# lab-oak/oak

Measured on AMD Instinct MI355X. Metric: turn-steps/s (batched playouts), higher is better.
Workload: dtype u16

## Files before the change

### include/oakgpu.h

```cpp
#ifndef OAKGPU_H
#define OAKGPU_H
#include <stddef.h>
#include <stdint.h>

#ifdef __cplusplus
extern "C" {
#endif

#define OAKGPU_BATTLE_SIZE 384
#define OAKGPU_DURATIONS_SIZE 8
#define OAKGPU_ACTIONS_SIZE 16
#define OAKGPU_MAX_CHOICES 9
#define OAKGPU_TEAMS_SIZE 60

typedef struct oakgpu_ctx oakgpu_ctx;
typedef struct oakgpu_net oakgpu_net;

int oakgpu_create(oakgpu_ctx **out, int device);
void oakgpu_destroy(oakgpu_ctx *ctx);
const char *oakgpu_last_error(void);
int oakgpu_set_stream(oakgpu_ctx *ctx, void *hip_stream);
void *oakgpu_get_stream(oakgpu_ctx *ctx);
int oakgpu_synchronize(oakgpu_ctx *ctx);
int oakgpu_set_kernel_timing(oakgpu_ctx *ctx, int on);
int oakgpu_get_leaf_kernel_ms(oakgpu_ctx *ctx, float ms[3]);
int oakgpu_set_playouts_per_lane(oakgpu_ctx *ctx, int k);
int oakgpu_set_regroup(oakgpu_ctx *ctx, int rounds, int suspend_below, int shrink);
int oakgpu_set_tail_pack(oakgpu_ctx *ctx, int below, int waves, int lanes);
int oakgpu_set_queue_order(oakgpu_ctx *ctx, int on);
int oakgpu_set_spread(oakgpu_ctx *ctx, int lanes);
int oakgpu_set_migration(oakgpu_ctx *ctx, int mode, int long_steps, int adopters);
int oakgpu_set_migration_window(oakgpu_ctx *ctx, int window);
int oakgpu_set_standstill_skip(oakgpu_ctx *ctx, int on);
#define OAKGPU_MOVE_CARRY_DEFAULT 32
int oakgpu_set_move_carry(oakgpu_ctx *ctx, int below);
#define OAKGPU_CTL_FAST_FORWARDED 44
#define OAKGPU_CTL_SKIPPED_STEPS 45
int oakgpu_get_queue_counters(oakgpu_ctx *ctx, uint32_t *out64);
int oakgpu_device_count(void);

int oakgpu_rollout_dev(oakgpu_ctx *ctx, const uint8_t *battles, const uint8_t *durations,
                       const uint8_t *results_in, uint8_t *prng_state, uint32_t n, uint32_t max_steps,
                       int prep, uint8_t *results_out, uint32_t *steps_out, float *values_out,
                       uint8_t *battles_out, uint8_t *durations_out);
int oakgpu_rollout(oakgpu_ctx *ctx, const uint8_t *battles, const uint8_t *durations,
                   const uint8_t *results_in, uint8_t *prng_state, uint32_t n, uint32_t max_steps, int prep,
                   uint8_t *results_out, uint32_t *steps_out, float *values_out, uint8_t *battles_out,
                   uint8_t *durations_out);

typedef struct {
  const uint8_t *battles, *durations, *results_in;
  uint8_t *prng_state;
  uint32_t n;
  uint8_t *results_out;
  uint32_t *steps_out;
  float *values_out;
  uint8_t *battles_out, *durations_out;
} oakgpu_rollout_batch;
// ... 434 lines not shown
```

### oak_amd/_lib.py

```python
import ctypes as C
import os

_HERE = os.path.dirname(os.path.abspath(__file__))
LIB_PATH = os.environ.get("OAKGPU_LIB") or os.path.join(_HERE, "liboakgpu.so")

SYMBOLS = [
    "oakgpu_create", "oakgpu_destroy", "oakgpu_last_error", "oakgpu_set_stream", "oakgpu_get_stream", "oakgpu_synchronize", "oakgpu_set_kernel_timing", "oakgpu_get_leaf_kernel_ms", "oakgpu_set_playouts_per_lane", "oakgpu_set_regroup", "oakgpu_set_tail_pack", "oakgpu_set_queue_order", "oakgpu_queue_order", "oakgpu_set_spread", "oakgpu_set_migration", "oakgpu_set_migration_window", "oakgpu_set_standstill_skip", "oakgpu_set_move_carry", "oakgpu_get_queue_counters",
    "oakgpu_device_count", "oakgpu_rollout_dev", "oakgpu_rollout", "oakgpu_rollout_group_dev", "oakgpu_rollout_group",
    "oakgpu_mt19937_fill", "oakgpu_rollout_draws_dev", "oakgpu_rollout_shared_device", "oakgpu_update_dev", "oakgpu_update",
    "oakgpu_choices_dev", "oakgpu_choices", "oakgpu_init_battles_dev", "oakgpu_init_battles",
    "oakgpu_set_ou_pools", "oakgpu_random_ou_battles_dev",
    "oakgpu_net_load", "oakgpu_net_load_memory", "oakgpu_net_free", "oakgpu_net_shape", "oakgpu_net_set_main_precision", "oakgpu_net_main_precision", "oakgpu_net_policy_form",
    "oakgpu_net_load_discrete", "oakgpu_net_load_discrete_memory", "oakgpu_net_is_discrete", "oakgpu_leaf_eval_discrete_raw_dev",
    "oakgpu_leaf_eval_dev", "oakgpu_leaf_eval", "oakgpu_leaf_eval_cached_dev", "oakgpu_leaf_cache_last_count", "oakgpu_leaf_embed_forms", "oakgpu_leaf_eval_policy_dev", "oakgpu_leaf_eval_policy",
    "oakgpu_heap_create", "oakgpu_heap_destroy", "oakgpu_heap_empty", "oakgpu_heap_clear", "oakgpu_heap_kind", "oakgpu_heap_nodes", "oakgpu_heap_update",
    "oakgpu_heap_root_stats", "oakgpu_heap_child_stats", "oakgpu_search_heap", "oakgpu_search_agent_heap", "oakgpu_heap_check_shards", "oakgpu_heap_selftest",
    "oakgpu_tree_step_dev", "oakgpu_search", "oakgpu_search_many", "oakgpu_search_agent", "oakgpu_agent_networks_clear", "oakgpu_bandit_replay", "oakgpu_bandit_select_run", "oakgpu_solve_matrix",
    "oakgpu_segment_mean_dev", "oakgpu_comm_unique_id", "oakgpu_comm_create", "oakgpu_comm_destroy", "oakgpu_all_gather_dev",
    "oakgpu_root_steps_create", "oakgpu_root_steps_destroy", "oakgpu_root_steps_launch_dev", "oakgpu_root_steps_capacity", "oakgpu_root_steps_reserve",
    "oakgpu_endless_battle_check", "oakgpu_frames_size", "oakgpu_frames_write", "oakgpu_frames_read", "oakgpu_selfplay_game", "oakgpu_selfplay_games", "oakgpu_poke_engine_eval_dev", "oakgpu_poke_engine_eval",
    "oakgpu_replay_index", "oakgpu_replay_records_dev", "oakgpu_replay_records", "oakgpu_engine_switches",
    "oakgpu_corpus_create", "oakgpu_corpus_destroy", "oakgpu_corpus_info", "oakgpu_frames_encode_dev", "oakgpu_frames_sample_dev", "oakgpu_encode_battles_dev",
    "oakgpu_frames_encode", "oakgpu_frames_sample",
    "oakgpu_corpus_frame_bases", "oakgpu_corpus_chunks", "oakgpu_corpus_states_dev", "oakgpu_corpus_states", "oakgpu_corpus_inference_dev", "oakgpu_corpus_loss_dev",
    "oakgpu_corpus_inference", "oakgpu_corpus_evaluate",
    "oakgpu_party_table_create", "oakgpu_party_table_destroy", "oakgpu_party_table_fill_dev", "oakgpu_party_table_fill", "oakgpu_leaf_eval_table_dev",
    "oakgpu_leaf_eval_policy_table_dev", "oakgpu_party_table_last_misses", "oakgpu_party_table_rows", "oakgpu_party_table_width", "oakgpu_party_key", "oakgpu_party_variant",
    "oakgpu_set_search_party_table", "oakgpu_search_party_table_stats", "oakgpu_leaf_eval_table", "oakgpu_leaf_eval_policy_table",
    "oakgpu_policy_games_dev", "oakgpu_policy_games", "oakgpu_policy_games_last_stats",
    "oakgpu_forest_create", "oakgpu_forest_destroy", "oakgpu_forest_check", "oakgpu_forest_search_dev", "oakgpu_forest_search", "oakgpu_forest_nodes",
# ... 137 lines not shown
                          "(hipcc --offload-arch=gfx950); there is no CPU fallback")
    lib = C.CDLL(LIB_PATH)
    vp, u32, u64, i32 = C.c_void_p, C.c_uint32, C.c_uint64, C.c_int
    lib.oakgpu_create.argtypes = [C.POINTER(vp), i32]
    lib.oakgpu_destroy.argtypes = [vp]
    lib.oakgpu_destroy.restype = None
    lib.oakgpu_last_error.restype = C.c_char_p
    lib.oakgpu_set_stream.argtypes = [vp, vp]
    lib.oakgpu_get_stream.argtypes = [vp]
    lib.oakgpu_get_stream.restype = vp
    lib.oakgpu_synchronize.argtypes = [vp]
    lib.oakgpu_set_kernel_timing.argtypes = [vp, i32]
    lib.oakgpu_get_leaf_kernel_ms.argtypes = [vp, C.POINTER(C.c_float)]
    lib.oakgpu_set_playouts_per_lane.argtypes = [vp, i32]
    lib.oakgpu_set_regroup.argtypes = [vp, i32, i32, i32]
    lib.oakgpu_set_tail_pack.argtypes = [vp, i32, i32, i32]
    lib.oakgpu_set_queue_order.argtypes = [vp, i32]
    lib.oakgpu_queue_order.argtypes = [vp, C.POINTER(RolloutBatch), u32, vp, C.POINTER(u32)]
    lib.oakgpu_set_spread.argtypes = [vp, i32]
    lib.oakgpu_set_migration.argtypes = [vp, i32, i32, i32]
    lib.oakgpu_set_migration_window.argtypes = [vp, i32]
    lib.oakgpu_set_standstill_skip.argtypes = [vp, i32]
    lib.oakgpu_set_move_carry.argtypes = [vp, i32]
    lib.oakgpu_get_queue_counters.argtypes = [vp, vp]
    lib.oakgpu_rollout_dev.argtypes = [vp, vp, vp, vp, vp, u32, u32, i32, vp, vp, vp, vp, vp]
    lib.oakgpu_rollout.argtypes = [vp, vp, vp, vp, vp, u32, u32, i32, vp, vp, vp, vp, vp]
    lib.oakgpu_rollout_group_dev.argtypes = [vp, C.POINTER(RolloutBatch), u32, u32, i32]
    lib.oakgpu_rollout_group.argtypes = [vp, C.POINTER(RolloutBatch), u32, u32, i32]
    lib.oakgpu_mt19937_fill.argtypes = [u32, u64, vp, C.c_size_t]
    lib.oakgpu_rollout_draws_dev.argtypes = [vp, vp, u32, vp, u32, vp, u32, vp, u32, vp, u32, u32, i32, vp, vp, vp, vp, vp, vp]
    lib.oakgpu_rollout_shared_device.argtypes = [vp, vp, vp, C.c_uint8, vp, u32, u32, u32, i32, vp, vp, vp, vp, vp, vp, vp]
    lib.oakgpu_poke_engine_eval_dev.argtypes = [vp, vp, u32, C.c_float, vp, vp]
    lib.oakgpu_poke_engine_eval.argtypes = [vp, vp, u32, C.c_float, vp, vp]
    lib.oakgpu_tree_step_dev.argtypes = [vp, vp, vp, vp, vp, vp, u32, u32, vp, vp, vp, vp, vp]
    lib.oakgpu_search.argtypes = [vp, vp, vp, vp, C.c_uint8, C.POINTER(SearchParams), C.POINTER(SearchOutput)]
    lib.oakgpu_heap_create.argtypes = [C.POINTER(vp)]
    lib.oakgpu_heap_destroy.argtypes = [vp]
    lib.oakgpu_heap_destroy.restype = None
    lib.oakgpu_heap_empty.argtypes = [vp]
    lib.oakgpu_heap_clear.argtypes = [vp]
    lib.oakgpu_heap_clear.restype = None
    lib.oakgpu_heap_kind.argtypes = [vp]
    lib.oakgpu_heap_nodes.argtypes = [vp]
    lib.oakgpu_heap_nodes.restype = u64
    lib.oakgpu_heap_update.argtypes = [vp, C.c_uint8, C.c_uint8, vp]
    lib.oakgpu_heap_root_stats.argtypes = [vp, i32, vp, vp, vp, vp]
# ... 146 lines not shown
```

### oak_amd/csrc/gen1_regs.hpp

```cpp
#pragma once
#include "gen1_device.hpp"

namespace oak {

#ifdef OAKGPU_SITE_PROFILE
static __device__ unsigned long long g_site_prof[32 * 4];
__device__ __forceinline__ unsigned long long *site_lds() {
  __shared__ unsigned long long s_prof[32 * 4];
  return s_prof;
}
__device__ __forceinline__ void site_zero() {
  unsigned long long *p = site_lds();
  for (int i = threadIdx.x; i < 32 * 4; i += blockDim.x) p[i] = 0;
  __syncthreads();
}
__device__ __forceinline__ void site_flush() {
  __syncthreads();
  unsigned long long *p = site_lds();
  for (int i = threadIdx.x; i < 32 * 4; i += blockDim.x) if (p[i]) atomicAdd(&g_site_prof[i], p[i]);
}
__device__ __forceinline__ void site_add(int id, long long dt) {
  const uint64_t ex = __ballot(1);
  const uint32_t lane = __lane_id();
  if ((ex & ((1ull << lane) - 1)) == 0) {
// ... 33 lines not shown
struct SideR {
  uint32_t a0, a1, a2;
  uint32_t bo;
  uint32_t vlo, vhi;
  uint32_t m01, m23;
  uint32_t p0, p1, p2, p3, p4, p5;
  uint32_t o0, o1;
  uint32_t dur;
  uint32_t misc;
};

#define OAK_FOR_SIDE_FIELDS(X) X(a0) X(a1) X(a2) X(bo) X(vlo) X(vhi) X(m01) X(m23) X(p0) X(p1) X(p2) X(p3) X(p4) X(p5) X(o0) X(o1) X(dur) X(misc)

__device__ __forceinline__ void swap_sides(SideR &a, SideR &b) {
#define X(f) asm("v_swap_b32 %0, %1" : "+v"(a.f), "+v"(b.f));
  OAK_FOR_SIDE_FIELDS(X)
#undef X
}
__device__ __forceinline__ void cswap_sides(bool c, SideR &a, SideR &b) {
#define X(f) { uint32_t t = c ? b.f : a.f; b.f = c ? a.f : b.f; a.f = t; }
  OAK_FOR_SIDE_FIELDS(X)
#undef X
}

template <int STRIDE, bool TRACK_ACTIONS, bool GIN_LDS = false>
struct EngineR {
  lds_u32 *m;
  Tables T;
  SideR S, F;
  uint64_t actS, actF;
#ifdef OAKGPU_SITE_PROFILE
  int prof_k = 0;
#endif
  uint64_t rng;
  uint32_t turn, last_damage;
  uint32_t lm;

  static constexpr int PARTY_WORDS = 24;
  template <bool L, class Dummy = void> struct GinPtr { typedef const uint32_t *type; };
  template <class Dummy> struct GinPtr<true, Dummy> { typedef const lds_u32 *type; };
  typedef typename GinPtr<GIN_LDS>::type gin_t;
  gin_t gin;
  __device__ __forceinline__ uint4 gin4(int off) const {
    typedef uint32_t v4 __attribute__((ext_vector_type(4)));
    if constexpr (GIN_LDS) { const v4 t = *(const OAK_LDS v4 *)(gin + off); return make_uint4(t.x, t.y, t.z, t.w); }
    else return *(const uint4 *)(gin + off);
// ... 155 lines not shown
#pragma unroll
    for (uint32_t sd = 0; sd < 2; ++sd)
#pragma unroll
      for (uint32_t i = 0; i < 6; ++i) {
        const uint32_t d2 = gdw(sd, i, 2), d3 = gdw(sd, i, 3), d4 = gdw(sd, i, 4), d5 = gdw(sd, i, 5);
        set_pw(sd, i, 0, pack_pp(d2, d3, d4));
        set_pw(sd, i, 1, (d4 >> 16) | ((d5 & 0xFF) << 16));
      }
    { const uint4 v = gin4(36); S.a0 = v.x; S.a1 = v.y; S.a2 = v.z; S.bo = v.w; }
    { const uint4 v = gin4(40); S.vlo = v.x; S.vhi = v.y; S.m01 = v.z; S.m23 = v.w; }
    S.o0 = gin[44]; S.o1 = gin[45];
    F.a0 = gin[82]; F.a1 = gin[83];
    { const uint4 v = gin4(84); F.a2 = v.x; F.bo = v.y; F.vlo = v.z; F.vhi = v.w; }
    { const uint4 v = gin4(88); F.m01 = v.x; F.m23 = v.y; F.o0 = v.z; F.o1 = v.w; }
    { const uint4 v = gin4(92); turn = v.x & 0xFFFF; last_damage = v.x >> 16; lm = v.y; rng = (uint64_t)v.z | ((uint64_t)v.w << 32); }
    S.dur = dur0; F.dur = dur1;
    S.misc = 0; F.misc = 1u << 8;
    actS = actF = 0;
    alive_from_lds(S);
    alive_from_lds(F);
    load_stored(S);
    load_stored(F);
  }
  __device__ __forceinline__ void store_battle_global(uint8_t *battle384) {
    if (order0(S) != 0) writeback_stored(S);
    if (order0(F) != 0) writeback_stored(F);
    uint32_t *g = (uint32_t *)battle384;
#pragma unroll
    for (uint32_t sd = 0; sd < 2; ++sd)
#pragma unroll
      for (uint32_t i = 0; i < 6; ++i) {
        const uint32_t pp = pw(sd, i, 0), hs = pw(sd, i, 1);
        uint32_t *d = g + sd * 46 + i * 6;
        d[0] = gdw(sd, i, 0);
        d[1] = gdw(sd, i, 1);
        d[2] = (gdw(sd, i, 2) & 0x00FFFFFFu) | ((pp & 0xFF) << 24);
        d[3] = (gdw(sd, i, 3) & 0x00FF00FFu) | (((pp >> 8) & 0xFF) << 8) | (((pp >> 16) & 0xFF) << 24);
        d[4] = (gdw(sd, i, 4) & 0x000000FFu) | ((pp >> 24) << 8) | ((hs & 0xFFFF) << 16);
        d[5] = (gdw(sd, i, 5) & 0xFFFFFF00u) | ((hs >> 16) & 0xFF);
      }
    *(uint4 *)(g + 36) = make_uint4(S.a0, S.a1, S.a2, S.bo);
    *(uint4 *)(g + 40) = make_uint4(S.vlo, S.vhi, S.m01, S.m23);
    g[44] = S.o0; g[45] = S.o1;
    g[82] = F.a0; g[83] = F.a1;
    *(uint4 *)(g + 84) = make_uint4(F.a2, F.bo, F.vlo, F.vhi);
    *(uint4 *)(g + 88) = make_uint4(F.m01, F.m23, F.o0, F.o1);
    *(uint4 *)(g + 92) = make_uint4(turn | (last_damage << 16), lm, (uint32_t)rng, (uint32_t)(rng >> 32));
// ... 774 lines not shown
  __device__ __forceinline__ uint32_t end_turn() {
    turn += 1;
    if (turn >= 1000) return mk_result(R_TIE, 0, 0);
    return mk_result(0, C_MOVE, C_MOVE);
  }

  __device__ __forceinline__ void normalize() {
    const bool flipped = absp(S) != 0;
    cswap_sides(flipped, S, F);
    if constexpr (TRACK_ACTIONS) { uint64_t t = flipped ? actF : actS; actF = flipped ? actS : actF; actS = t; }
  }

  __device__ __forceinline__ uint32_t post_action(uint32_t choice, bool replace, bool residual) {
    OAK_SCOPE(PS_FAINT_RESIDUAL);
    if (replace) return 0;
    uint32_t r = 0;
    if ((choice & 3) != C_SWITCH) r = check_faint(F, S);
    if (r == 0) {
      if (residual) handle_residual();
      r = check_faint(S, F);
    }
    return r;
  }
  __device__ __forceinline__ uint32_t act_cheap(uint32_t choice) {
    const bool replace = hp(S) == 0;
    if ((choice & 3) == C_SWITCH) { OAK_SCOPE(PS_SWITCH_IN); switch_in(S, F, choice >> 2); }
    return post_action(choice, replace, false);
  }
  __device__ __forceinline__ uint32_t act_move(uint32_t choice) {
    OAK_T0(t_em);
    const bool replace = hp(S) == 0;
    uint32_t mslot = choice >> 2;
    if (last_sel(S) == M_Struggle) mslot = 0;
    else if (mslot == 0) mslot = lm_index(absp(S));
    OAK_T0(t_bm);
    const int r = before_move();
    OAK_T1(PS_BEFORE_MOVE, t_bm);
    if (r == BM_ERR) return mk_result(R_ERROR, 0, 0);
    if (r != BM_DONE) execute_selected(mslot, r == BM_SKIP_CAN, r == BM_SKIP_PP);
    OAK_T1(PS_EXEC_MOVE, t_em);
    OAK_T1K(PS_EXEC_MOVE_K0, t_em);
    return post_action(choice, replace, true);
  }

  __device__ __forceinline__ uint32_t turn_prologue(uint32_t cS, uint32_t cF, uint32_t &pc, uint32_t &qc) {
    if constexpr (TRACK_ACTIONS) { actS = 0; actF = 0; }
    if (turn == 0) {
      const bool aS = (S.misc & 63) != 0, aF = (F.misc & 63) != 0;
      const bool s_p1 = absp(S) == 0;
      if (!aS) return mk_result(aF ? (s_p1 ? R_LOSE : R_WIN) : R_TIE, 0, 0);
      if (!aF) return mk_result(s_p1 ? R_WIN : R_LOSE, 0, 0);
#pragma unroll 1
      for (int k = 0; k < 2; ++k) { switch_in(S, F, 1); swap_sides(S, F); }
      return end_turn();
    }
    OAK_T0(t_ord);
    select_move(S, cS);
    select_move(F, cF);
    bool f_first;
    {
      const uint32_t tS = cS & 3, tF = cF & 3;
      if (tS == C_PASS) f_first = true;
      else if (tF == C_PASS) f_first = false;
      else if ((tS == C_SWITCH) != (tF == C_SWITCH)) f_first = tS != C_SWITCH;
      else {
        const uint32_t mS = last_sel(S), mF = last_sel(F);
        bool decided = false;
        f_first = false;
        if (tS == C_MOVE) {
          if ((mS == M_QuickAttack) != (mF == M_QuickAttack)) { f_first = mS != M_QuickAttack; decided = true; }
          else if ((mS == M_Counter) != (mF == M_Counter)) { f_first = mS == M_Counter; decided = true; }
        }
        if (!decided) {
          const uint32_t sS = spe(S), sF = spe(F);
          if (sS == sF) {
            const bool p1 = rng_range(0, 2) == 0;
            act_set(true, AC_SPEEDTIE, 2, p1 ? 1 : 2);
            act_set(false, AC_SPEEDTIE, 2, p1 ? 1 : 2);
            f_first = p1 != (absp(S) == 0);
          } else f_first = sS < sF;
        }
      }
    }
    pc = f_first ? cF : cS;
    qc = f_first ? cS : cF;
    cswap_sides(f_first, S, F);
    if constexpr (TRACK_ACTIONS) { uint64_t t = f_first ? actF : actS; actF = f_first ? actS : actF; actS = t; }
    OAK_T1(PS_ORDER, t_ord);
    return 0;
  }
  __device__ __forceinline__ uint32_t turn_epilogue() {
    if ((S.vlo & V_BINDING) && attacks(S) == 0) clear_binding(S);
    if ((F.vlo & V_BINDING) && attacks(F) == 0) clear_binding(F);
    return end_turn();
  }
  __device__ __forceinline__ void next_actor() {
    swap_sides(S, F);
    if constexpr (TRACK_ACTIONS) { uint64_t t = actS; actS = actF; actF = t; }
  }

  __device__ __forceinline__ uint32_t act(uint32_t choice) { return (choice & 3) == C_MOVE ? act_move(choice) : act_cheap(choice); }
  __device__ __forceinline__ void hand_over(uint32_t &pc, uint32_t &qc) {
    next_actor();
    const uint32_t t = pc; pc = qc; qc = t;
  }
  __device__ __forceinline__ uint32_t turn_finish(uint32_t r) { return r ? r : turn_epilogue(); }

  __device__ uint32_t update_frame(uint32_t cS, uint32_t cF) {
    uint32_t pc = 0, qc = 0;
    uint32_t r = turn_prologue(cS, cF, pc, qc);
    if (r) return r;
#pragma unroll 1
    for (int k = 0; k < 2; ++k) {
      OAK_SET_K(*this, k);
      r = act(pc);
      const bool last = r != 0 || (qc & 3) == C_PASS;
      hand_over(pc, qc);
      if (last) break;
    }
    return turn_finish(r);
  }
  __device__ __forceinline__ uint32_t update(uint32_t c1, uint32_t c2) {
    const uint32_t r = update_frame(c1, c2);
    normalize();
// ... 171 lines not shown
```

### oak_amd/csrc/oakgpu.hip

```cpp
#include <hip/hip_runtime.h>
#include <stdint.h>
#include <stdio.h>
#include <stdlib.h>
#include <string.h>
#include <algorithm>
#include <random>
#include <mutex>
#include <string>
#include <type_traits>
#include <vector>

#include "../../include/oakgpu.h"
#include "gen1_device.hpp"
#include "gen1_regs.hpp"
#include "record_walk.hpp"
#include "oakgpu_internal.h"
#include "fast_prng.hpp"

namespace oak {
using namespace walk;

constexpr int STATE_WORDS = 96;
constexpr int TABLE_LDS_PAD = TABLE_PAD;

// ... 251 lines not shown
  if (a.battles_out) e.store_battle_global(a.battles_out + (size_t)lane * 384);
}

struct RoundArgs {
  const uint32_t *list_in;
  const uint32_t *n_in;
  uint32_t *list_out;
  uint32_t *count_out;
  uint8_t *sb;
  uint8_t *sd;
  uint8_t *sres;
  uint32_t suspend_below;
  uint32_t *queue;
  uint32_t lanes;
  const uint32_t *order;
  uint32_t *adopt_ctl;
  uint64_t *adopt_list;
  uint32_t epoch;
  uint32_t n_adopters;
  uint32_t long_steps;
  uint32_t no_skip;
  uint32_t *stats;
  uint32_t move_carry;
};

struct BatchDesc {
  const uint8_t *battles, *durations, *results_in;
  uint8_t *prng;
  uint8_t *results_out;
  uint32_t *steps_out;
  float *values_out;
  uint8_t *battles_out, *durations_out;
  uint32_t start, n;
};
constexpr int MAX_GROUP = 64;
struct GroupArgs {
  const BatchDesc *table;
  uint32_t count, total, max_steps;
  int prep;
};

struct ColdArgs {
  GroupArgs g;
  RoundArgs q;
  uint32_t starts[MAX_GROUP];
};
// ... 86 lines not shown
#define OAK_PRIO_STILL 24
#endif
constexpr uint32_t PRIO_STILL = OAK_PRIO_STILL;
template <int BLK, int WPS>
__global__ __launch_bounds__(BLK, WPS) void k_rollout_queue(GroupArgs g_in, RoundArgs q_in) {
  extern __shared__ __align__(16) uint8_t smem[];
  lds_u32 *party = (lds_u32 *)smem;
  using ER = EngineR<BLK, false>;
  Tables T = stage_default_tables((lds_u8 *)smem + ER::PARTY_WORDS * BLK * 4);
  lds_u32 *cold = (lds_u32 *)((lds_u8 *)smem + ER::PARTY_WORDS * BLK * 4 + TABLE_LDS_PAD);
  if (threadIdx.x == 0) {
    struct { GroupArgs g; RoundArgs q; } c{g_in, q_in};
    const uint32_t *src = (const uint32_t *)&c;
#pragma unroll
    for (uint32_t i = 0; i < offsetof(ColdArgs, starts) / 4; ++i) cold[i] = src[i];
  }
  for (uint32_t i = threadIdx.x; i < g_in.count; i += BLK) cold[offsetof(ColdArgs, starts) / 4 + i] = g_in.table[i].start;
  __syncthreads();
  const uint32_t tid = threadIdx.x, wl = tid & 63;
  constexpr uint32_t NONE = 0xFFFFFFFFu, DONE = 0xFFFFFFFEu;
#define COLD_U32(off) ((uint32_t)__builtin_amdgcn_readfirstlane((int)cold[(off) / 4]))
#define COLD_QU(field) COLD_U32(offsetof(ColdArgs, q) + offsetof(RoundArgs, field))
#define COLD_GU(field) COLD_U32(offsetof(ColdArgs, g) + offsetof(GroupArgs, field))
  constexpr uint32_t U_RESUME = 1, U_PREP = 2, U_ADOPTER = 4, U_DRY = 8, U_ADOPTING = 16, U_ANY_PLAYING = 32, U_NO_SKIP = 64;
  uint32_t ust = (COLD_QU(list_in) | COLD_U32(offsetof(ColdArgs, q) + offsetof(RoundArgs, list_in) + 4)) != 0 ? U_RESUME : 0u;
#define IS_RESUME ((ust & U_RESUME) != 0)
#define IS_PREP ((ust & U_PREP) != 0)
  const uint32_t total = IS_RESUME ? (uint32_t)__builtin_amdgcn_readfirstlane((int)*COLD_Q(n_in, const uint32_t *)) : COLD_GU(total);
  const uint32_t max_steps = COLD_GU(max_steps), suspend_below = COLD_QU(suspend_below);
  if (!IS_RESUME && COLD_GU(prep) != 0) ust |= U_PREP;
  ust |= (blockIdx.x & 7u) << 8;
  if (COLD_QU(no_skip) != 0) ust |= U_NO_SKIP;
  if (!IS_RESUME && COLD_QU(lanes) == 0) ust |= (COLD_QU(move_carry) & 0xFFu) << 24;
  ER e;
  e.m = party + tid;
  e.T = T;
  FastPrng g;
  g.s0 = g.s1 = 0;
  uint32_t idx = NONE, result = 0, steps = 0;
  { const uint32_t lanes = COLD_QU(lanes); if (lanes && wl >= lanes) idx = DONE; }
#define IS_DRY ((ust & U_DRY) != 0)
  const uint32_t n_adopt = COLD_QU(n_adopters), long_steps = COLD_QU(long_steps);
  uint32_t stale = 0;
  if (n_adopt != 0 && blockIdx.x < n_adopt) ust |= U_ADOPTER;
#define IS_ADOPTER ((ust & U_ADOPTER) != 0)
#define IS_ADOPTING ((ust & U_ADOPTING) != 0)
#define ANY_PLAYING ((ust & U_ANY_PLAYING) != 0)
  uint32_t idle_polls = 0, poll_tick = 15;
  constexpr uint32_t SPIN_CAP = 1u << 22;
  constexpr int ERR_WORD = 23;
  OAK_PROF_ZERO();
  OAK_TL(0, wall_clock64());
#ifdef OAKGPU_TIMELINE
  bool tl_dry = false;
  unsigned long long tl_steps = 0;
#endif
  for (;;) {
    bool need = idx == NONE, load = false, from_scratch = IS_RESUME;
    uint64_t mask = __ballot(need);
    if (mask && IS_ADOPTER && ((++poll_tick & 15u) == 0 || !ANY_PLAYING)) {
      uint32_t *ctl = COLD_Q(adopt_ctl, uint32_t *);
      uint32_t h = 0, k = 0, closed = 0;
      if (wl == 0) {
        for (int tries = 0; tries < 8; ++tries) {
          const uint32_t hh = __hip_atomic_load(ctl + 1, __ATOMIC_ACQUIRE, __HIP_MEMORY_SCOPE_AGENT);
          const uint32_t t = __hip_atomic_load(ctl + 0, __ATOMIC_ACQUIRE, __HIP_MEMORY_SCOPE_AGENT);
          if (t) closed |= 2;
          const uint32_t kk = t > hh ? min(t - hh, (uint32_t)__popcll(mask)) : 0u;
          if (!kk) {
            if (__hip_atomic_load(ctl + 2, __ATOMIC_ACQUIRE, __HIP_MEMORY_SCOPE_AGENT) == gridDim.x - n_adopt &&
                __hip_atomic_load(ctl + 0, __ATOMIC_ACQUIRE, __HIP_MEMORY_SCOPE_AGENT) == hh &&
                __hip_atomic_load(ctl + 1, __ATOMIC_ACQUIRE, __HIP_MEMORY_SCOPE_AGENT) == hh) closed |= 1;
            break;
          }
          if (atomicCAS(ctl + 1, hh, hh + kk) == hh) { h = hh; k = kk; break; }
        }
      }
      h = (uint32_t)__builtin_amdgcn_readfirstlane((int)h); k = (uint32_t)__builtin_amdgcn_readfirstlane((int)k); closed = (uint32_t)__builtin_amdgcn_readfirstlane((int)closed);
      if (closed & 2) ust |= U_ADOPTING;
      const uint32_t rank = (uint32_t)__popcll(mask & ((1ull << wl) - 1));
      const bool take = need && rank < k;
      uint32_t got = 0;
      if (take && h + rank < COLD_GU(total)) {
        const uint64_t *slot = COLD_Q(adopt_list, const uint64_t *) + h + rank;
        const uint32_t epoch = COLD_QU(epoch);
        uint32_t spins = 0;
        uint64_t tk;
        while ((uint32_t)((tk = __hip_atomic_load(slot, __ATOMIC_RELAXED, __HIP_MEMORY_SCOPE_AGENT)) >> 32) != epoch && ++spins < SPIN_CAP) __builtin_amdgcn_s_sleep(2);
        if ((uint32_t)(tk >> 32) == epoch) got = (uint32_t)tk;
        if (!got) atomicOr(ctl + ERR_WORD, 1u);
      }
      if (k) __builtin_amdgcn_fence(__ATOMIC_ACQUIRE, "agent");
      if (take && got) { idx = got - 1; load = true; from_scratch = true; }
// ... 68 lines not shown
    if (start && stale >= (8u << 24) && !(ust & U_NO_SKIP)) {
      const int draws = e.inert_standstill(result);
      const uint32_t by_steps = max_steps - steps, by_turn = 1000u - e.turn;
      const uint32_t skip = (by_steps < by_turn ? by_steps : by_turn) - 1u;
      if (draws >= 0 && skip != 0) {
        for (uint32_t k = 0; k < skip; ++k) { (void)g.next32(); (void)g.next32(); }
        e.rng_jump((uint32_t)draws * skip);
        e.turn += skip;
        steps += skip;
        atomicAdd((unsigned long long *)COLD_Q(stats, uint32_t *), 1ull | ((unsigned long long)skip << 32));
      }
    }
    {
      OAK_SCOPE(PS_STEP);
      if (start) {
        OAK_T0(t_ld);
        const uint32_t hi = g.next32(), lo = g.next32();
        uint32_t cS, cF, pc = 0, qc = 0;
        e.random_choices(result, hi, lo, cS, cF);
        OAK_T1(PS_LEGAL_DRAW, t_ld);
        const uint32_t r = e.turn_prologue(cS, cF, pc, qc);
        result = r ? (r | T_DONE) : (T_PEND | (pc << 16) | (qc << 24));
      }
      const bool carrying = (ust >> 24) != 0 && !(ust & (U_DRY | U_ADOPTING));
#pragma unroll 1
      for (uint32_t walk = carrying ? 0u : 1u;; ++walk) {
        const uint32_t c = (result >> 16) & 0xFFu;
        if ((result & T_PEND) && (walk != 0 || (c & 3) != C_MOVE)) {
          OAK_SET_K(e, walk ? walk - 1 : 0);
          const uint32_t r = e.act(c);
          e.next_actor();
          const uint32_t next = T_PEND | ((result >> 8) & 0xFF0000u);
          result = (r != 0 || ((next >> 16) & 3) == C_PASS) ? (r | T_DONE) : next;
        }
        if (walk == 2) break;
        if (walk == 1) {
          const uint32_t want = (uint32_t)__popcll(__ballot((result & T_PEND) != 0));
          if (want == 0 || (carrying && want < (ust >> 24))) break;
        }
      }
      if (result & T_DONE) {
        result = e.turn_finish(result & 0xFFu);
        ++steps;
        playing = (result & 15) == 0 && steps < max_steps;
        const uint32_t sg = ((e.S.p4 ^ e.F.p4) >> 16) | (((e.S.o0 + e.F.o0) & 0xFFu) << 16);
        stale = sg != (stale & 0xFFFFFFu) ? sg : stale + (stale < 0xFF000000u ? 0x01000000u : 0u);
      }
    }
    if (IS_ADOPTING || __ballot(playing && (steps > LONG_STEPS || stale >= (PRIO_STILL << 24)))) __builtin_amdgcn_s_setprio(3); else __builtin_amdgcn_s_setprio(0);
    if (__ballot(playing) != 0) ust |= U_ANY_PLAYING; else ust &= ~U_ANY_PLAYING;
    if (IS_ADOPTER && !ANY_PLAYING) {
      __builtin_amdgcn_s_sleep(100);
      if (++idle_polls > SPIN_CAP) { if (wl == 0) atomicOr(COLD_Q(adopt_ctl, uint32_t *) + ERR_WORD, 2u); break; }
    }
    const uint64_t still = __ballot(playing);
    const bool suspend = IS_DRY && still != 0 && (uint32_t)__popcll(still) < suspend_below;
    const bool lng = n_adopt != 0 && !IS_ADOPTER && playing && !(result & T_PEND) && (steps >= (long_steps & 0xFFFFu) || (stale >> 24) >= (long_steps >> 16));
    if (idx != DONE && idx != NONE && (!playing || suspend || lng)) {
      OAK_SCOPE(PS_PUBLISH);
      const bool fin = !playing;
      e.normalize();
      const BatchDesc *bd = find_batch(cold, idx);
      const uint32_t k = idx - bd->start;
      if (fin) bd->results_out[k] = (uint8_t)result; else COLD_Q(sres, uint8_t *)[idx] = (uint8_t)result;
      bd->steps_out[k] = steps;
      const uint32_t t = result & 15;
      if (fin) bd->values_out[k] = t == R_WIN ? 1.0f : t == R_LOSE ? 0.0f : 0.5f;
      uint32_t *pdst = (uint32_t *)bd->prng + 2 * (size_t)k;
      pdst[0] = g.s0;
      pdst[1] = g.s1;
      uint32_t *ddst = fin ? (bd->durations_out ? (uint32_t *)bd->durations_out + 2 * (size_t)k : nullptr) : COLD_Q(sd, uint32_t *) + 2 * (size_t)idx;
      if (ddst) {
        ddst[0] = e.S.dur;
        ddst[1] = e.F.dur;
      }
      uint8_t *bdst = fin ? (bd->battles_out ? bd->battles_out + (size_t)k * 384 : nullptr) : COLD_Q(sb, uint8_t *) + (size_t)idx * 384;
      if (bdst) e.store_battle_global(bdst);
      idx = fin ? NONE : idx;
    }
    const uint64_t dm = __ballot(lng);
    if (dm) {
      __builtin_amdgcn_fence(__ATOMIC_RELEASE, "agent");
      uint32_t *ctl = COLD_Q(adopt_ctl, uint32_t *);
      const uint32_t leader = (uint32_t)__ffsll((unsigned long long)dm) - 1;
      uint32_t base = 0;
      if (wl == leader) base = atomicAdd(ctl + 0, (uint32_t)__popcll(dm));
      base = (uint32_t)__builtin_amdgcn_readlane((int)base, (int)leader);
      if (lng) {
        __hip_atomic_store(COLD_Q(adopt_list, uint64_t *) + base + (uint32_t)__popcll(dm & ((1ull << wl) - 1)), (uint64_t)(idx + 1) | ((uint64_t)COLD_QU(epoch) << 32),
                           __ATOMIC_RELAXED, __HIP_MEMORY_SCOPE_AGENT);
        idx = NONE;
      }
    }
    if (suspend) {
      const uint32_t leader = (uint32_t)__ffsll((unsigned long long)still) - 1;
      uint32_t base = 0;
      if (wl == leader) base = atomicAdd(COLD_Q(count_out, uint32_t *), (uint32_t)__popcll(still));
      base = (uint32_t)__builtin_amdgcn_readlane((int)base, (int)leader);
      if (playing) COLD_Q(list_out, uint32_t *)[base + (uint32_t)__popcll(still & ((1ull << wl) - 1))] = idx;
      break;
    }
  }
  if (n_adopt != 0 && !IS_ADOPTER && wl == 0) atomicAdd(COLD_Q(adopt_ctl, uint32_t *) + 2, 1u);
  OAK_TL(2, wall_clock64());
#ifdef OAKGPU_TIMELINE
  OAK_TL(4, tl_steps);
#endif
  OAK_PROF_FLUSH();
}
#undef COLD_Q
#undef COLD_U32
#undef COLD_QU
#undef COLD_GU
#undef IS_RESUME
#undef IS_PREP
#undef IS_DRY
#undef IS_ADOPTER
#undef IS_ADOPTING
#undef ANY_PLAYING

struct RootStepArgs {
  const uint8_t *root_battles, *root_durations, *root_results;
  uint8_t *lane_prng;
  const uint4 *cin_state;
  const uint32_t *cin_count;
  uint4 *cout_state;
  uint32_t *cout_count;
  unsigned long long *acc;
  unsigned long long *turn_steps;
  uint32_t *queue;
  uint32_t *err;
  uint32_t n_fresh, reps, seg, slice_mask, max_steps, fper;
  uint32_t acc_stride, pad;
};
#ifndef OAK_ROOT_REFILL_EVERY
#define OAK_ROOT_REFILL_EVERY 8
#endif
#ifndef OAK_ROOT_REFILL_LANES
#define OAK_ROOT_REFILL_LANES 16
#endif
constexpr uint32_t ROOT_REFILL_EVERY = OAK_ROOT_REFILL_EVERY, ROOT_REFILL_LANES = OAK_ROOT_REFILL_LANES;
constexpr int ROOT_SHARDS = 8;
// ... 615 lines not shown
  uint32_t *d_heads;
  int rounds;
  int suspend_below;
  int round_shrink;
  uint8_t *d_scratch;
  size_t scratch_n;
  int rounds_auto;
  int concurrent_hint;
  int search_party_table;
  uint64_t search_table_fills = 0, search_table_evals = 0;
  const void *ws2_owner = nullptr;
  int tail_below;
  int tail_waves;
  int tail_lanes;
  int migrate;
  int migrate_steps;
  int migrate_adopters;
  int migrate_window;
  int migrate_used;
  int spread_lanes;
  int queue_order;
  int standstill_skip;
  int move_carry;
  uint32_t *d_order;
  size_t order_n;
  uint32_t order_pair = 0;
  uint32_t ticket_epoch = 0;
  bool tickets_dirty = true;
  int n_cu;
  static constexpr int TABLE_SLOTS = 8;
  void *h_table, *d_table;
  hipEvent_t table_ev[TABLE_SLOTS];
  uint64_t table_next;
  struct Block { void *p; size_t cap; };
  std::vector<Block> stage;
  size_t stage_cursor;
  Block ws[3];
  int timing;
  hipEvent_t tev[4];
  bool tev_valid;
  Block replay_ws{nullptr, 0};
  Block games_ws{nullptr, 0};
  void *attachment = nullptr;
  void (*attachment_dtor)(void *) = nullptr;
};

// ... 144 lines not shown
  if (const char *env = getenv("OAKGPU_PARTY_TABLE")) c->search_party_table = atoi(env) != 0;
  if (const char *env = getenv("OAKGPU_ROUNDS_AUTO")) c->rounds_auto = atoi(env) != 0;
  {
    hipDeviceProp_t prop;
    hipError_t pe = hipGetDeviceProperties(&prop, device);
    if (pe != hipSuccess) { delete c; return fail(pe, "hipGetDeviceProperties"); }
    c->n_cu = prop.multiProcessorCount > 0 ? prop.multiProcessorCount : 256;
  }
  c->rounds = 4;
  c->suspend_below = 32;
  c->round_shrink = 3;
  c->tail_below = 0;
  c->tail_waves = 0;
  if (const char *env = getenv("OAKGPU_TAIL_BELOW")) c->tail_below = atoi(env) < 0 ? 0 : atoi(env) > 64 ? 64 : atoi(env);
  if (const char *env = getenv("OAKGPU_TAIL_WAVES")) c->tail_waves = atoi(env) < 0 ? 0 : atoi(env);
  c->spread_lanes = -1;
  if (const char *env = getenv("OAKGPU_SPREAD_LANES")) c->spread_lanes = atoi(env) < -1 ? -1 : atoi(env) > 64 ? 64 : atoi(env);
  c->queue_order = 1;
  if (const char *env = getenv("OAKGPU_QUEUE_ORDER")) c->queue_order = atoi(env) != 0;
  c->standstill_skip = 1;
  if (const char *env = getenv("OAKGPU_STANDSTILL_SKIP")) c->standstill_skip = atoi(env) != 0;
  c->move_carry = OAKGPU_MOVE_CARRY_DEFAULT;
  if (const char *env = getenv("OAKGPU_MOVE_CARRY")) c->move_carry = atoi(env) < 0 ? 0 : atoi(env) > 64 ? 64 : atoi(env);
  c->migrate = 1;
  c->migrate_steps = 300;
  c->migrate_adopters = 0;
  c->migrate_window = 48;
  c->migrate_used = 0;
  if (const char *env = getenv("OAKGPU_MIGRATE")) c->migrate = atoi(env) < 0 ? 0 : atoi(env) > 2 ? 2 : atoi(env);
  if (const char *env = getenv("OAKGPU_MIGRATE_STEPS")) c->migrate_steps = atoi(env) < 1 ? 1 : atoi(env);
  if (const char *env = getenv("OAKGPU_MIGRATE_ADOPTERS")) c->migrate_adopters = atoi(env) < 0 ? 0 : atoi(env);
  if (const char *env = getenv("OAKGPU_MIGRATE_WINDOW")) c->migrate_window = atoi(env) < 0 ? 0 : atoi(env) > 255 ? 255 : atoi(env);
  c->d_order = nullptr;
  c->order_n = 0;
  c->tail_lanes = 0;
  if (const char *env = getenv("OAKGPU_TAIL_LANES")) c->tail_lanes = atoi(env) < 0 ? 0 : atoi(env) > 64 ? 64 : atoi(env);
  if (const char *env = getenv("OAKGPU_ROUNDS")) c->rounds = atoi(env) < 1 ? 1 : atoi(env) > 8 ? 8 : atoi(env);
  if (const char *env = getenv("OAKGPU_SUSPEND_BELOW")) c->suspend_below = atoi(env) < 0 ? 0 : atoi(env) > 64 ? 64 : atoi(env);
  if (const char *env = getenv("OAKGPU_ROUND_SHRINK")) c->round_shrink = atoi(env) < 1 ? 1 : atoi(env);
  hipError_t e = hipStreamCreateWithFlags(&c->stream, hipStreamNonBlocking);
  if (e != hipSuccess) { delete c; return fail(e, "hipStreamCreate"); }
  *out = c;
  return 0;
}

void oakgpu_destroy(oakgpu_ctx *c) {
// ... 67 lines not shown
  HIPCHK(hipMemcpyAsync(out64, c->d_queue, 256, hipMemcpyDeviceToHost, c->stream));
  HIPCHK(hipStreamSynchronize(c->stream));
  return 0;
}

int oakgpu_set_spread(oakgpu_ctx *c, int lanes) {
  if (!c || lanes < -1 || lanes > 64) return bad("oakgpu_set_spread: lanes must be -1 (automatic) or 0..64");
  c->spread_lanes = lanes;
  return 0;
}

int oakgpu_set_standstill_skip(oakgpu_ctx *c, int on) {
  if (!c) return bad("null ctx");
  c->standstill_skip = on != 0;
  return 0;
}

int oakgpu_set_move_carry(oakgpu_ctx *c, int below) {
  if (!c || below < 0 || below > 64) return bad("oakgpu_set_move_carry: below must be 0 (off) .. 64 lanes");
  c->move_carry = below;
  return 0;
}

int oakgpu_set_search_party_table(oakgpu_ctx *c, int on) {
  if (!c) return bad("null ctx");
  const int old = c->search_party_table;
  c->search_party_table = on != 0;
  return old;
}

int oakgpu_search_party_table_stats(oakgpu_ctx *c, uint64_t *fills, uint64_t *evals) {
  if (!c) return bad("null ctx");
  if (fills) *fills = c->search_table_fills;
  if (evals) *evals = c->search_table_evals;
  return 0;
}

int oakgpu_set_queue_order(oakgpu_ctx *c, int on) {
  if (!c) return bad("null ctx");
  c->queue_order = on != 0;
  return 0;
}

int oakgpu_set_tail_pack(oakgpu_ctx *c, int below, int waves, int lanes) {
  if (!c || below < 0 || below > 64 || waves < 0 || lanes < 0 || lanes > 64) return bad("oakgpu_set_tail_pack: bad argument");
  c->tail_below = below;
// ... 132 lines not shown
  }
  if (migrate) {
    if (++c->ticket_epoch == 0 || c->tickets_dirty) {
      HIPCHK(hipMemsetAsync(lists[0], 0, (size_t)c->scratch_n * 8, c->stream));
      if (c->ticket_epoch == 0) c->ticket_epoch = 1;
      c->tickets_dirty = false;
    }
    c->migrate_used = 1;
  } else if (rounds > 1) c->tickets_dirty = true;
  for (int r = 0; r < rounds; ++r) {
    oak::RoundArgs q{};
    q.order = r == 0 ? order : nullptr;
    q.long_steps = (uint32_t)(c->migrate_steps > 0xFFFF ? 0xFFFF : c->migrate_steps) | (uint32_t)(c->migrate_window > 0 ? c->migrate_window : 256) << 16;
    q.no_skip = c->standstill_skip ? 0u : 1u;
    q.move_carry = (uint32_t)c->move_carry;
    q.stats = c->d_queue + OAKGPU_CTL_FAST_FORWARDED;
    if (migrate) { q.adopt_ctl = c->d_queue + 40; q.adopt_list = (uint64_t *)lists[0]; q.epoch = c->ticket_epoch; q.n_adopters = adopters; }
    q.list_in = r ? lists[(r - 1) & 1] : nullptr;
    q.n_in = r ? c->d_queue + 2 * r - 1 : nullptr;
    q.list_out = lists[r & 1];
    q.count_out = c->d_queue + 2 * r + 1;
    q.sb = sb; q.sd = sd; q.sres = sres;
    q.suspend_below = r + 1 < rounds ? (uint32_t)(tail_pack ? c->tail_below : c->suspend_below) : 0u;
    q.queue = c->d_heads + (size_t)r * oak::QUEUE_HEADS * oak::QUEUE_HEAD_STRIDE;
    q.lanes = (tail_pack && r > 0) ? (uint32_t)c->tail_lanes : (r == 0 ? spread : 0u);
    hipLaunchKernelGGL((oak::k_rollout_queue<64, 4>), dim3(waves), dim3(64), lq, c->stream, g, q);
    waves = tail_pack ? (uint32_t)(c->tail_waves > 0 ? c->tail_waves : c->n_cu) : (waves + c->round_shrink - 1) / c->round_shrink;
    if (waves < 1) waves = 1;
  }
  HIPCHK(hipGetLastError());
  return 0;
}

int oakgpu_queue_order(oakgpu_ctx *c, const oakgpu_rollout_batch *batches, uint32_t count, uint32_t *order_out, uint32_t *suspects_out) {
  if (!c || !batches || !order_out || count == 0 || count > (uint32_t)oak::MAX_GROUP) return bad("oakgpu_queue_order: bad argument");
  HIPCHK(hipSetDevice(c->device));
  uint64_t total = 0;
  for (uint32_t i = 0; i < count; ++i) { if (!batches[i].battles || batches[i].n == 0) return bad("oakgpu_queue_order: empty batch"); total += batches[i].n; }
  if (total >= 0xFFFFFFF0ull) return bad("oakgpu_queue_order: more than 2^32 playouts");
  uint8_t *d_battles = nullptr;
  HIPCHK(hipMalloc((void **)&d_battles, (size_t)total * 384));
  oak::BatchDesc descs[oak::MAX_GROUP] = {};
  uint32_t start = 0;
  int rc = 0;
  for (uint32_t i = 0; i < count && !rc; ++i) {
    descs[i].battles = d_battles + (size_t)start * 384;
// ... 622 lines not shown
```

### oak_amd/engine.py

```python
import ctypes as C
import os

import numpy as np

from . import _lib, gamedata


def _p(a):
    return None if a is None else a.ctypes.data_as(C.c_void_p)


def _u8(a, shape=None):
    a = np.ascontiguousarray(a, dtype=np.uint8)
    return a if shape is None else a.reshape(shape)


class Context:

    def __init__(self, device=0):
        self.lib = _lib.load()
        h = C.c_void_p()
        _lib.check(self.lib.oakgpu_create(C.byref(h), device))
        self.handle = h
        self.device = device
# ... 33 lines not shown
    def set_migration_window(self, window=48):
        _lib.check(self.lib.oakgpu_set_migration_window(self.handle, int(window)))

    def set_search_party_table(self, on=True):
        return bool(self.lib.oakgpu_set_search_party_table(self.handle, int(bool(on))))

    def search_party_table_stats(self):
        fills, evals = C.c_uint64(), C.c_uint64()
        _lib.check(self.lib.oakgpu_search_party_table_stats(self.handle, C.byref(fills), C.byref(evals)))
        return fills.value, evals.value

    def queue_order(self, battles_per_batch):
        bs = [_u8(b) for b in battles_per_batch]
        descs = (_lib.RolloutBatch * len(bs))()
        for k, b in enumerate(bs):
            descs[k].battles, descs[k].n = b.ctypes.data, b.shape[0]
        order = np.zeros(sum(b.shape[0] for b in bs), dtype=np.uint32)
        suspects = C.c_uint32(0)
        _lib.check(self.lib.oakgpu_queue_order(self.handle, descs, len(bs), _p(order), C.byref(suspects)))
        return order, suspects.value

    def set_move_carry(self, below=0):
        _lib.check(self.lib.oakgpu_set_move_carry(self.handle, int(below)))

    def set_standstill_skip(self, on=True):
        _lib.check(self.lib.oakgpu_set_standstill_skip(self.handle, 1 if on else 0))

    def queue_counters(self):
        out = np.zeros(64, dtype=np.uint32)
        _lib.check(self.lib.oakgpu_get_queue_counters(self.handle, out.ctypes.data_as(C.c_void_p)))
        return out


    def stream_ptr(self):
        return self.lib.oakgpu_get_stream(self.handle)

    def synchronize(self):
        _lib.check(self.lib.oakgpu_synchronize(self.handle))

    def ensure_ou_pools(self):
        if not self._pools:
            legal, pools, sizes = gamedata.ou_pools()
            _lib.check(self.lib.oakgpu_set_ou_pools(self.handle, _p(legal), len(legal),
                                                    _p(np.ascontiguousarray(pools)), _p(sizes)))
            self._pools = True

# ... 211 lines not shown
```

Measured before the change: 10.82 billion.

## Add opt-in move carry for dry waves and trim rollout kernel register state

Adds a move_carry_dry setting, off by default, that lets dry (queue-exhausted) waves keep carrying move actions when enough lanes are still playing, and skips suspension for those waves. Merges act_move and act_cheap into a single act function, and replaces cswap_sides with a branch on f_first. Publishing now maps sides to players by copying into new P1/P2 structs instead of calling normalize() in place. The migration flag is kept in a bit of ust instead of a live n_adopt register, and n_adopters is reread from the kernel args where it is needed, which is meant to lower register pressure at the cost of some extra scalar loads and code churn.

```diff
diff --git a/include/oakgpu.h b/include/oakgpu.h
--- a/include/oakgpu.h
+++ b/include/oakgpu.h
@@ -34,6 +34,8 @@
 int oakgpu_set_standstill_skip(oakgpu_ctx *ctx, int on);
 #define OAKGPU_MOVE_CARRY_DEFAULT 32
 int oakgpu_set_move_carry(oakgpu_ctx *ctx, int below);
+#define OAKGPU_MOVE_CARRY_DRY_DEFAULT 0
+int oakgpu_set_move_carry_dry(oakgpu_ctx *ctx, int below);
 #define OAKGPU_CTL_FAST_FORWARDED 44
 #define OAKGPU_CTL_SKIPPED_STEPS 45
 int oakgpu_get_queue_counters(oakgpu_ctx *ctx, uint32_t *out64);
diff --git a/oak_amd/_lib.py b/oak_amd/_lib.py
--- a/oak_amd/_lib.py
+++ b/oak_amd/_lib.py
@@ -5,7 +5,7 @@
 LIB_PATH = os.environ.get("OAKGPU_LIB") or os.path.join(_HERE, "liboakgpu.so")
 
 SYMBOLS = [
-    "oakgpu_create", "oakgpu_destroy", "oakgpu_last_error", "oakgpu_set_stream", "oakgpu_get_stream", "oakgpu_synchronize", "oakgpu_set_kernel_timing", "oakgpu_get_leaf_kernel_ms", "oakgpu_set_playouts_per_lane", "oakgpu_set_regroup", "oakgpu_set_tail_pack", "oakgpu_set_queue_order", "oakgpu_queue_order", "oakgpu_set_spread", "oakgpu_set_migration", "oakgpu_set_migration_window", "oakgpu_set_standstill_skip", "oakgpu_set_move_carry", "oakgpu_get_queue_counters",
+    "oakgpu_create", "oakgpu_destroy", "oakgpu_last_error", "oakgpu_set_stream", "oakgpu_get_stream", "oakgpu_synchronize", "oakgpu_set_kernel_timing", "oakgpu_get_leaf_kernel_ms", "oakgpu_set_playouts_per_lane", "oakgpu_set_regroup", "oakgpu_set_tail_pack", "oakgpu_set_queue_order", "oakgpu_queue_order", "oakgpu_set_spread", "oakgpu_set_migration", "oakgpu_set_migration_window", "oakgpu_set_standstill_skip", "oakgpu_set_move_carry", "oakgpu_set_move_carry_dry", "oakgpu_get_queue_counters",
     "oakgpu_device_count", "oakgpu_rollout_dev", "oakgpu_rollout", "oakgpu_rollout_group_dev", "oakgpu_rollout_group",
     "oakgpu_mt19937_fill", "oakgpu_rollout_draws_dev", "oakgpu_rollout_shared_device", "oakgpu_update_dev", "oakgpu_update",
     "oakgpu_choices_dev", "oakgpu_choices", "oakgpu_init_battles_dev", "oakgpu_init_battles",
@@ -189,6 +189,7 @@
     lib.oakgpu_set_migration_window.argtypes = [vp, i32]
     lib.oakgpu_set_standstill_skip.argtypes = [vp, i32]
     lib.oakgpu_set_move_carry.argtypes = [vp, i32]
+    lib.oakgpu_set_move_carry_dry.argtypes = [vp, i32]
     lib.oakgpu_get_queue_counters.argtypes = [vp, vp]
     lib.oakgpu_rollout_dev.argtypes = [vp, vp, vp, vp, vp, u32, u32, i32, vp, vp, vp, vp, vp]
     lib.oakgpu_rollout.argtypes = [vp, vp, vp, vp, vp, u32, u32, i32, vp, vp, vp, vp, vp]
diff --git a/oak_amd/csrc/gen1_regs.hpp b/oak_amd/csrc/gen1_regs.hpp
--- a/oak_amd/csrc/gen1_regs.hpp
+++ b/oak_amd/csrc/gen1_regs.hpp
@@ -79,6 +79,11 @@
   OAK_FOR_SIDE_FIELDS(X)
 #undef X
 }
+__device__ __forceinline__ void sides_by_player(bool c, const SideR &a, const SideR &b, SideR &p1, SideR &p2) {
+#define X(f) p1.f = c ? b.f : a.f; p2.f = c ? a.f : b.f;
+  OAK_FOR_SIDE_FIELDS(X)
+#undef X
+}
 
 template <int STRIDE, bool TRACK_ACTIONS, bool GIN_LDS = false>
 struct EngineR {
@@ -280,7 +285,8 @@
     load_stored(S);
     load_stored(F);
   }
-  __device__ __forceinline__ void store_battle_global(uint8_t *battle384) {
+  __device__ __forceinline__ void store_battle_global(uint8_t *battle384) { store_battle_global(battle384, S, F); }
+  __device__ __forceinline__ void store_battle_global(uint8_t *battle384, const SideR &S, const SideR &F) {
     if (order0(S) != 0) writeback_stored(S);
     if (order0(F) != 0) writeback_stored(F);
     uint32_t *g = (uint32_t *)battle384;
@@ -1101,26 +1107,6 @@
     }
     return r;
   }
-  __device__ __forceinline__ uint32_t act_cheap(uint32_t choice) {
-    const bool replace = hp(S) == 0;
-    if ((choice & 3) == C_SWITCH) { OAK_SCOPE(PS_SWITCH_IN); switch_in(S, F, choice >> 2); }
-    return post_action(choice, replace, false);
-  }
-  __device__ __forceinline__ uint32_t act_move(uint32_t choice) {
-    OAK_T0(t_em);
-    const bool replace = hp(S) == 0;
-    uint32_t mslot = choice >> 2;
-    if (last_sel(S) == M_Struggle) mslot = 0;
-    else if (mslot == 0) mslot = lm_index(absp(S));
-    OAK_T0(t_bm);
-    const int r = before_move();
-    OAK_T1(PS_BEFORE_MOVE, t_bm);
-    if (r == BM_ERR) return mk_result(R_ERROR, 0, 0);
-    if (r != BM_DONE) execute_selected(mslot, r == BM_SKIP_CAN, r == BM_SKIP_PP);
-    OAK_T1(PS_EXEC_MOVE, t_em);
-    OAK_T1K(PS_EXEC_MOVE_K0, t_em);
-    return post_action(choice, replace, true);
-  }
 
   __device__ __forceinline__ uint32_t turn_prologue(uint32_t cS, uint32_t cF, uint32_t &pc, uint32_t &qc) {
     if constexpr (TRACK_ACTIONS) { actS = 0; actF = 0; }
@@ -1163,7 +1149,7 @@
     }
     pc = f_first ? cF : cS;
     qc = f_first ? cS : cF;
-    cswap_sides(f_first, S, F);
+    if (f_first) swap_sides(S, F);
     if constexpr (TRACK_ACTIONS) { uint64_t t = f_first ? actF : actS; actF = f_first ? actS : actF; actS = t; }
     OAK_T1(PS_ORDER, t_ord);
     return 0;
@@ -1178,7 +1164,23 @@
     if constexpr (TRACK_ACTIONS) { uint64_t t = actS; actS = actF; actF = t; }
   }
 
-  __device__ __forceinline__ uint32_t act(uint32_t choice) { return (choice & 3) == C_MOVE ? act_move(choice) : act_cheap(choice); }
+  __device__ __forceinline__ uint32_t act(uint32_t choice) {
+    const uint32_t hp0 = hp(S);
+    if ((choice & 3) == C_MOVE) {
+      OAK_T0(t_em);
+      uint32_t mslot = choice >> 2;
+      if (last_sel(S) == M_Struggle) mslot = 0;
+      else if (mslot == 0) mslot = lm_index(absp(S));
+      OAK_T0(t_bm);
+      const int r = before_move();
+      OAK_T1(PS_BEFORE_MOVE, t_bm);
+      if (r == BM_ERR) return mk_result(R_ERROR, 0, 0);
+      if (r != BM_DONE) execute_selected(mslot, r == BM_SKIP_CAN, r == BM_SKIP_PP);
+      OAK_T1(PS_EXEC_MOVE, t_em);
+      OAK_T1K(PS_EXEC_MOVE_K0, t_em);
+    } else if ((choice & 3) == C_SWITCH) { OAK_SCOPE(PS_SWITCH_IN); switch_in(S, F, choice >> 2); }
+    return post_action(choice, hp0 == 0, (choice & 3) == C_MOVE);
+  }
   __device__ __forceinline__ void hand_over(uint32_t &pc, uint32_t &qc) {
     next_actor();
     const uint32_t t = pc; pc = qc; qc = t;
diff --git a/oak_amd/csrc/oakgpu.hip b/oak_amd/csrc/oakgpu.hip
--- a/oak_amd/csrc/oakgpu.hip
+++ b/oak_amd/csrc/oakgpu.hip
@@ -297,6 +297,7 @@
   uint32_t no_skip;
   uint32_t *stats;
   uint32_t move_carry;
+  uint32_t move_carry_dry;
 };
 
 struct BatchDesc {
@@ -429,7 +430,7 @@
 #define COLD_U32(off) ((uint32_t)__builtin_amdgcn_readfirstlane((int)cold[(off) / 4]))
 #define COLD_QU(field) COLD_U32(offsetof(ColdArgs, q) + offsetof(RoundArgs, field))
 #define COLD_GU(field) COLD_U32(offsetof(ColdArgs, g) + offsetof(GroupArgs, field))
-  constexpr uint32_t U_RESUME = 1, U_PREP = 2, U_ADOPTER = 4, U_DRY = 8, U_ADOPTING = 16, U_ANY_PLAYING = 32, U_NO_SKIP = 64;
+  constexpr uint32_t U_RESUME = 1, U_PREP = 2, U_ADOPTER = 4, U_DRY = 8, U_ADOPTING = 16, U_ANY_PLAYING = 32, U_NO_SKIP = 64, U_CARRIED = 128, U_MIGRATE = 1u << 11;
   uint32_t ust = (COLD_QU(list_in) | COLD_U32(offsetof(ColdArgs, q) + offsetof(RoundArgs, list_in) + 4)) != 0 ? U_RESUME : 0u;
 #define IS_RESUME ((ust & U_RESUME) != 0)
 #define IS_PREP ((ust & U_PREP) != 0)
@@ -447,9 +448,9 @@
   uint32_t idx = NONE, result = 0, steps = 0;
   { const uint32_t lanes = COLD_QU(lanes); if (lanes && wl >= lanes) idx = DONE; }
 #define IS_DRY ((ust & U_DRY) != 0)
-  const uint32_t n_adopt = COLD_QU(n_adopters), long_steps = COLD_QU(long_steps);
+  const uint32_t long_steps = COLD_QU(long_steps);
   uint32_t stale = 0;
-  if (n_adopt != 0 && blockIdx.x < n_adopt) ust |= U_ADOPTER;
+  { const uint32_t n_adopt = COLD_QU(n_adopters); if (n_adopt != 0) ust |= blockIdx.x < n_adopt ? U_MIGRATE | U_ADOPTER : U_MIGRATE; }
 #define IS_ADOPTER ((ust & U_ADOPTER) != 0)
 #define IS_ADOPTING ((ust & U_ADOPTING) != 0)
 #define ANY_PLAYING ((ust & U_ANY_PLAYING) != 0)
@@ -475,7 +476,7 @@
           if (t) closed |= 2;
           const uint32_t kk = t > hh ? min(t - hh, (uint32_t)__popcll(mask)) : 0u;
           if (!kk) {
-            if (__hip_atomic_load(ctl + 2, __ATOMIC_ACQUIRE, __HIP_MEMORY_SCOPE_AGENT) == gridDim.x - n_adopt &&
+            if (__hip_atomic_load(ctl + 2, __ATOMIC_ACQUIRE, __HIP_MEMORY_SCOPE_AGENT) == gridDim.x - COLD_QU(n_adopters) &&
                 __hip_atomic_load(ctl + 0, __ATOMIC_ACQUIRE, __HIP_MEMORY_SCOPE_AGENT) == hh &&
                 __hip_atomic_load(ctl + 1, __ATOMIC_ACQUIRE, __HIP_MEMORY_SCOPE_AGENT) == hh) closed |= 1;
             break;
@@ -590,9 +591,14 @@
         const uint32_t r = e.turn_prologue(cS, cF, pc, qc);
         result = r ? (r | T_DONE) : (T_PEND | (pc << 16) | (qc << 24));
       }
-      const bool carrying = (ust >> 24) != 0 && !(ust & (U_DRY | U_ADOPTING));
+      if ((ust >> 24) != 0 && !(ust & (U_DRY | U_ADOPTING))) ust |= U_CARRIED; else ust &= ~U_CARRIED;
+      if ((ust >> 24) != 0 && IS_DRY && !IS_ADOPTER) {
+        const uint32_t dry_below = COLD_QU(move_carry_dry);
+        if (dry_below != 0 && (uint32_t)__popcll(__ballot(playing)) >= dry_below) ust |= U_CARRIED;
+      }
+#define CARRYING ((ust & U_CARRIED) != 0)
 #pragma unroll 1
-      for (uint32_t walk = carrying ? 0u : 1u;; ++walk) {
+      for (uint32_t walk = CARRYING ? 0u : 1u;; ++walk) {
         const uint32_t c = (result >> 16) & 0xFFu;
         if ((result & T_PEND) && (walk != 0 || (c & 3) != C_MOVE)) {
           OAK_SET_K(e, walk ? walk - 1 : 0);
@@ -604,7 +610,7 @@
         if (walk == 2) break;
         if (walk == 1) {
           const uint32_t want = (uint32_t)__popcll(__ballot((result & T_PEND) != 0));
-          if (want == 0 || (carrying && want < (ust >> 24))) break;
+          if (want == 0 || (CARRYING && want < (ust >> 24))) break;
         }
       }
       if (result & T_DONE) {
@@ -622,12 +628,13 @@
       if (++idle_polls > SPIN_CAP) { if (wl == 0) atomicOr(COLD_Q(adopt_ctl, uint32_t *) + ERR_WORD, 2u); break; }
     }
     const uint64_t still = __ballot(playing);
-    const bool suspend = IS_DRY && still != 0 && (uint32_t)__popcll(still) < suspend_below;
-    const bool lng = n_adopt != 0 && !IS_ADOPTER && playing && !(result & T_PEND) && (steps >= (long_steps & 0xFFFFu) || (stale >> 24) >= (long_steps >> 16));
+    const bool suspend = IS_DRY && !(ust & U_CARRIED) && still != 0 && (uint32_t)__popcll(still) < suspend_below;
+    const bool lng = (ust & U_MIGRATE) != 0 && !IS_ADOPTER && playing && !(result & T_PEND) && (steps >= (long_steps & 0xFFFFu) || (stale >> 24) >= (long_steps >> 16));
     if (idx != DONE && idx != NONE && (!playing || suspend || lng)) {
       OAK_SCOPE(PS_PUBLISH);
       const bool fin = !playing;
-      e.normalize();
+      SideR P1, P2;
+      sides_by_player(ER::absp(e.S) != 0, e.S, e.F, P1, P2);
       const BatchDesc *bd = find_batch(cold, idx);
       const uint32_t k = idx - bd->start;
       if (fin) bd->results_out[k] = (uint8_t)result; else COLD_Q(sres, uint8_t *)[idx] = (uint8_t)result;
@@ -639,11 +646,11 @@
       pdst[1] = g.s1;
       uint32_t *ddst = fin ? (bd->durations_out ? (uint32_t *)bd->durations_out + 2 * (size_t)k : nullptr) : COLD_Q(sd, uint32_t *) + 2 * (size_t)idx;
       if (ddst) {
-        ddst[0] = e.S.dur;
-        ddst[1] = e.F.dur;
+        ddst[0] = P1.dur;
+        ddst[1] = P2.dur;
       }
       uint8_t *bdst = fin ? (bd->battles_out ? bd->battles_out + (size_t)k * 384 : nullptr) : COLD_Q(sb, uint8_t *) + (size_t)idx * 384;
-      if (bdst) e.store_battle_global(bdst);
+      if (bdst) e.store_battle_global(bdst, P1, P2);
       idx = fin ? NONE : idx;
     }
     const uint64_t dm = __ballot(lng);
@@ -669,7 +676,7 @@
       break;
     }
   }
-  if (n_adopt != 0 && !IS_ADOPTER && wl == 0) atomicAdd(COLD_Q(adopt_ctl, uint32_t *) + 2, 1u);
+  if ((ust & U_MIGRATE) != 0 && !IS_ADOPTER && wl == 0) atomicAdd(COLD_Q(adopt_ctl, uint32_t *) + 2, 1u);
   OAK_TL(2, wall_clock64());
 #ifdef OAKGPU_TIMELINE
   OAK_TL(4, tl_steps);
@@ -686,6 +693,7 @@
 #undef IS_ADOPTER
 #undef IS_ADOPTING
 #undef ANY_PLAYING
+#undef CARRYING
 
 struct RootStepArgs {
   const uint8_t *root_battles, *root_durations, *root_results;
@@ -1347,6 +1355,7 @@
   int queue_order;
   int standstill_skip;
   int move_carry;
+  int move_carry_dry;
   uint32_t *d_order;
   size_t order_n;
   uint32_t order_pair = 0;
@@ -1537,6 +1546,8 @@
   if (const char *env = getenv("OAKGPU_STANDSTILL_SKIP")) c->standstill_skip = atoi(env) != 0;
   c->move_carry = OAKGPU_MOVE_CARRY_DEFAULT;
   if (const char *env = getenv("OAKGPU_MOVE_CARRY")) c->move_carry = atoi(env) < 0 ? 0 : atoi(env) > 64 ? 64 : atoi(env);
+  c->move_carry_dry = OAKGPU_MOVE_CARRY_DRY_DEFAULT;
+  if (const char *env = getenv("OAKGPU_MOVE_CARRY_DRY")) c->move_carry_dry = atoi(env) < 0 ? 0 : atoi(env) > 64 ? 64 : atoi(env);
   c->migrate = 1;
   c->migrate_steps = 300;
   c->migrate_adopters = 0;
@@ -1650,6 +1661,12 @@
   return 0;
 }
 
+int oakgpu_set_move_carry_dry(oakgpu_ctx *c, int below) {
+  if (!c || below < 0 || below > 64) return bad("oakgpu_set_move_carry_dry: below must be 0 (off) .. 64 lanes");
+  c->move_carry_dry = below;
+  return 0;
+}
+
 int oakgpu_set_search_party_table(oakgpu_ctx *c, int on) {
   if (!c) return bad("null ctx");
   const int old = c->search_party_table;
@@ -1828,6 +1845,7 @@
     q.count_out = c->d_queue + 2 * r + 1;
     q.sb = sb; q.sd = sd; q.sres = sres;
     q.suspend_below = r + 1 < rounds ? (uint32_t)(tail_pack ? c->tail_below : c->suspend_below) : 0u;
+    q.move_carry_dry = c->move_carry_dry > 0 ? std::max((uint32_t)c->move_carry_dry, q.suspend_below) : 0u;
     q.queue = c->d_heads + (size_t)r * oak::QUEUE_HEADS * oak::QUEUE_HEAD_STRIDE;
     q.lanes = (tail_pack && r > 0) ? (uint32_t)c->tail_lanes : (r == 0 ? spread : 0u);
     hipLaunchKernelGGL((oak::k_rollout_queue<64, 4>), dim3(waves), dim3(64), lq, c->stream, g, q);
diff --git a/oak_amd/engine.py b/oak_amd/engine.py
--- a/oak_amd/engine.py
+++ b/oak_amd/engine.py
@@ -79,6 +79,9 @@
 
     def set_move_carry(self, below=0):
         _lib.check(self.lib.oakgpu_set_move_carry(self.handle, int(below)))
+
+    def set_move_carry_dry(self, below=0):
+        _lib.check(self.lib.oakgpu_set_move_carry_dry(self.handle, int(below)))
 
     def set_standstill_skip(self, on=True):
         _lib.check(self.lib.oakgpu_set_standstill_skip(self.handle, 1 if on else 0))
```

Measured after the change: 11.32 billion, median of 6. 1.05x the previous value.
